# UMEssen/Body-and-Organ-Analysis

Hardware: AMD Instinct MI355X
Metric: CT volumes/sec (512^3 @1.5 mm, total+bca) on MI355X (higher is better)
Workload: dtype f16

## Files before the change

body-and-organ-analysis_amd/csrc/api.hip:

```cpp
#include <stdarg.h>
#include <stdlib.h>
#include <algorithm>
#include <iterator>
#include <string.h>

#include "common.h"

static thread_local char g_err[1024] = "";

void boa_set_error(const char* fmt, ...) {
    va_list ap;
    va_start(ap, fmt);
    vsnprintf(g_err, sizeof(g_err), fmt, ap);
    va_end(ap);
}

extern "C" const char* boa_last_error(void) { return g_err; }
extern "C" int boa_version(void) { return 100; }

extern "C" int boa_init(int device, void* stream, boa_ctx** out) {
    BOA_REQUIRE(out != nullptr, "boa_init: out is NULL");
    int n = 0;
    BOA_HIP_TRY(hipGetDeviceCount(&n));
    BOA_REQUIRE(device >= 0 && device < n, "boa_init: device %d not available (%d visible)", device, n);
// ... 12 lines not shown
    for (int i = 0; i < 8; ++i) {
        BOA_HIP_TRY(hipEventCreate(&c->t0[i]));
        BOA_HIP_TRY(hipEventCreate(&c->t1[i]));
    }
    *out = c;
    return BOA_OK;
}

extern "C" void boa_destroy(boa_ctx* c) {
    if (!c) return;
    hipSetDevice(c->device);
    hipStreamSynchronize(c->stream);
    for (int i = 0; i < 8; ++i) {
        hipEventDestroy(c->t0[i]);
        hipEventDestroy(c->t1[i]);
    }
    for (auto& r : c->prof_pending) hipEventDestroy(r.ev);
    for (auto e : c->ev_pool) hipEventDestroy(e);
    for (auto& r : c->ws_runs) hipFree(r.second);
    for (auto& b : c->pool_free) hipFree(b.second);
    for (auto& b : c->pool_live) hipFree(b.first);
    if (c->stash) hipFree(c->stash);
    if (c->act_arena) hipFree(c->act_arena);
    if (c->own_stream) hipStreamDestroy(c->stream);
    delete c;
}

extern "C" int boa_device_info(boa_ctx* c, char* name, int name_len, int* cu_count, size_t* total_mem,
                               size_t* free_mem) {
    BOA_REQUIRE(c, "ctx is NULL");
    hipDeviceProp_t p;
    BOA_HIP_TRY(hipGetDeviceProperties(&p, c->device));
    if (name && name_len > 0) {
        snprintf(name, name_len, "%s (%s)", p.name, p.gcnArchName);
    }
    if (cu_count) *cu_count = p.multiProcessorCount;
    size_t f = 0, t = 0;
    BOA_HIP_TRY(hipMemGetInfo(&f, &t));
    if (total_mem) *total_mem = t;
    if (free_mem) *free_mem = f;
    return BOA_OK;
}

int boa_malloc_raw(boa_ctx* c, size_t bytes, void** dev_out) {
    BOA_REQUIRE(c && dev_out, "boa_malloc: NULL argument");
    BOA_HIP_TRY(hipSetDevice(c->device));
// ... 65 lines not shown
            BOA_HIP_TRY(hipFree(last->second));
            c->pool_bytes -= last->first;
            c->pool_free.erase(last);
        }
    }
    return BOA_OK;
}

static int trim_locked(boa_ctx* c);
extern "C" int boa_trim(boa_ctx* c) {
    BOA_REQUIRE(c, "ctx is NULL");
    std::lock_guard<std::recursive_mutex> lock(c->pool_mu);
    return trim_locked(c);
}

extern "C" int boa_bind_thread(boa_ctx* c) {
    BOA_REQUIRE(c, "ctx is NULL");
    BOA_HIP_TRY(hipSetDevice(c->device));
    return BOA_OK;
}

static int trim_locked(boa_ctx* c) {
    const bool drop_stash = c->stash && !c->stash_busy;
    if (c->pool_free.empty() && !drop_stash && c->ws_desc_bytes == 0) return BOA_OK;
    BOA_HIP_TRY(hipStreamSynchronize(c->stream));
    for (size_t i = c->ws_runs.size(); i-- > 0;)
        if (!c->ws_runs[i].first.empty() && c->ws_runs[i].first[0] == -1) {
            hipFree(c->ws_runs[i].second);
            c->ws_runs.erase(c->ws_runs.begin() + i);
            c->ws_runs_host.erase(c->ws_runs_host.begin() + i);
        }
    c->ws_desc_bytes = 0;
    for (auto& b : c->pool_free) hipFree(b.second);
    c->pool_free.clear();
    c->pool_bytes = 0;
    if (drop_stash) {
        hipFree(c->stash);
        c->stash = nullptr;
        c->stash_bytes = 0;
    }
    return BOA_OK;
}

extern "C" int boa_memset(boa_ctx* c, void* dev, int value, size_t bytes) {
    BOA_REQUIRE(c && dev, "boa_memset: NULL argument");
    KernelTimer t(c, BOA_K_OTHER, 0, (double)bytes);
    BOA_HIP_TRY(hipMemsetAsync(dev, value, bytes, c->stream));
    t.stop();
// ... 71 lines not shown

KernelTimer::KernelTimer(boa_ctx* c, int kclass, double flops, double bytes) : ctx(c), k(kclass) {
    if (!c->prof) return;
    if (c->prof_pending.size() >= 32768) boa_prof_flush(c);
    on = true;
    c->prof_flops[k] += flops;
    c->prof_bytes[k] += bytes;
    c->prof_launches[k] += 1;
    if (c->prof_break || c->prof_pending.empty()) {
        hipEvent_t e = take_event(c);
        hipEventRecord(e, c->stream);
        c->prof_pending.push_back({-1, e});
        c->prof_break = false;
    }
}

void KernelTimer::stop() {
    if (!on) return;
    hipEvent_t e = take_event(ctx);
    hipEventRecord(e, ctx->stream);
    ctx->prof_pending.push_back({k, e});
}

int boa_prof_flush(boa_ctx* c) {
    if (!c->prof_pending.empty()) hipEventSynchronize(c->prof_pending.back().ev);
    for (size_t i = 0; i < c->prof_pending.size(); ++i) {
        const ProfRec& r = c->prof_pending[i];
        float ms = 0.f;
        if (r.kclass >= 0 && i > 0 && hipEventElapsedTime(&ms, c->prof_pending[i - 1].ev, r.ev) == hipSuccess)
            c->prof_ms[r.kclass] += ms;
        c->ev_pool.push_back(r.ev);
    }
    c->prof_pending.clear();
    c->prof_break = true;
    return BOA_OK;
}

extern "C" long long boa_debug_counter(boa_ctx* c, int which, int reset) {
    if (!c || which < 0 || which >= BOA_CNT_COUNT) return -1;
    const long long v = c->counters[which];
    if (reset) c->counters[which] = 0;
    return v;
}

extern "C" int boa_prof_enable(boa_ctx* c, int on) {
    BOA_REQUIRE(c, "ctx is NULL");
    if (!on) boa_prof_flush(c);
    c->prof = on != 0;
    return BOA_OK;
}

extern "C" int boa_prof_reset(boa_ctx* c) {
    BOA_REQUIRE(c, "ctx is NULL");
    boa_prof_flush(c);
    for (int i = 0; i < BOA_K_COUNT; ++i) {
        c->prof_ms[i] = 0;
        c->prof_launches[i] = 0;
// ... 17 lines not shown
```

body-and-organ-analysis_amd/csrc/comm.hip:

```cpp
#include <dlfcn.h>
#include <stdlib.h>
#include <string.h>
#include <rccl/rccl.h>

#include <algorithm>
#include <string>

#include "common.h"

namespace {

struct Rccl {
    void* h = nullptr;
    ncclResult_t (*GetUniqueId)(ncclUniqueId*) = nullptr;
    ncclResult_t (*CommInitRank)(ncclComm_t*, int, ncclUniqueId, int) = nullptr;
    ncclResult_t (*CommDestroy)(ncclComm_t) = nullptr;
    ncclResult_t (*Send)(const void*, size_t, ncclDataType_t, int, ncclComm_t, hipStream_t) = nullptr;
    ncclResult_t (*Recv)(void*, size_t, ncclDataType_t, int, ncclComm_t, hipStream_t) = nullptr;
    ncclResult_t (*AllReduce)(const void*, void*, size_t, ncclDataType_t, ncclRedOp_t, ncclComm_t, hipStream_t) = nullptr;
    ncclResult_t (*GroupStart)() = nullptr;
    ncclResult_t (*GroupEnd)() = nullptr;
    const char* (*GetErrorString)(ncclResult_t) = nullptr;
    std::string path;
};
// ... 91 lines not shown
    BOA_REQUIRE(ctx && id_in && out && world >= 1 && rank >= 0 && rank < world, "boa_comm_create: bad argument (world %d, rank %d)", world, rank);
    Rccl* R = rccl();
    BOA_REQUIRE(R, "boa_comm: librccl.so not found (set BOA_RCCL_LIB)");
    BOA_HIP_TRY(hipSetDevice(ctx->device));
    boa_comm* c = new boa_comm;
    c->ctx = ctx;
    c->world = world;
    c->rank = rank;
    ncclUniqueId id;
    memcpy(&id, id_in, 128);
    ncclResult_t r = R->CommInitRank(&c->comm, world, id, rank);
    if (r != ncclSuccess) {
        boa_set_error("ncclCommInitRank(world %d, rank %d) failed: %s", world, rank, R->GetErrorString ? R->GetErrorString(r) : "?");
        delete c;
        return BOA_EHIP;
    }
    if (hipStreamCreateWithFlags(&c->stream, hipStreamNonBlocking) != hipSuccess || hipEventCreateWithFlags(&c->ev_in, hipEventDisableTiming) != hipSuccess ||
        hipEventCreateWithFlags(&c->ev_out, hipEventDisableTiming) != hipSuccess) {
        boa_set_error("boa_comm_create: stream / event creation failed");
        R->CommDestroy(c->comm);
        delete c;
        return BOA_EHIP;
    }
    *out = c;
    return BOA_OK;
}

extern "C" void boa_comm_destroy(boa_comm* c) {
    if (!c) return;
    Rccl* R = rccl();
    if (c->stream) hipStreamSynchronize(c->stream);
    if (R && c->comm) R->CommDestroy(c->comm);
    if (c->ev_in) hipEventDestroy(c->ev_in);
    if (c->ev_out) hipEventDestroy(c->ev_out);
    if (c->stream) hipStreamDestroy(c->stream);
    delete c;
}

static int fence_in(boa_comm* c) {
    BOA_HIP_TRY(hipEventRecord(c->ev_in, c->ctx->stream));
    BOA_HIP_TRY(hipStreamWaitEvent(c->stream, c->ev_in, 0));
    return BOA_OK;
}

static int fence_out(boa_comm* c) {
    BOA_HIP_TRY(hipEventRecord(c->ev_out, c->stream));
// ... 150 lines not shown
```

body-and-organ-analysis_amd/csrc/common.h:

```cpp
#pragma once
#include <hip/hip_runtime.h>
#include <hip/hip_fp16.h>
#include <stdint.h>
#include <stdio.h>
#include <map>
#include <unordered_map>
#include <mutex>
#include <vector>

#include "boa_hip.h"

void boa_set_error(const char* fmt, ...);

#define BOA_HIP_TRY(expr)                                                                       \
    do {                                                                                        \
        hipError_t _e = (expr);                                                                 \
        if (_e != hipSuccess) {                                                                 \
            boa_set_error("%s failed: %s (%s:%d)", #expr, hipGetErrorString(_e), __FILE__, __LINE__); \
            return (_e == hipErrorOutOfMemory) ? BOA_ENOMEM : BOA_EHIP;                         \
        }                                                                                       \
    } while (0)

#define BOA_REQUIRE(cond, ...)                \
    do {                                      \
        if (!(cond)) {                        \
            boa_set_error(__VA_ARGS__);       \
            return BOA_EINVAL;                \
        }                                     \
    } while (0)
// ... 18 lines not shown
    bool prof = false;
    bool prof_break = true;
    std::vector<ProfRec> prof_pending;
    std::vector<hipEvent_t> ev_pool;
    double prof_ms[BOA_K_COUNT] = {};
    long long prof_launches[BOA_K_COUNT] = {};
    double prof_flops[BOA_K_COUNT] = {};
    double prof_bytes[BOA_K_COUNT] = {};
    long long counters[BOA_CNT_COUNT] = {};
    std::vector<std::pair<std::vector<int>, void*>> ws_runs;
    std::vector<std::vector<int>> ws_runs_host;
    size_t ws_desc_bytes = 0;
    std::recursive_mutex pool_mu;
    std::multimap<size_t, void*> pool_free;
    std::unordered_map<void*, size_t> pool_live;
    size_t pool_bytes = 0;
    size_t pool_cap = 0;
    void* stash = nullptr;
    size_t stash_bytes = 0;
    bool stash_busy = false;
    void* act_arena = nullptr;
    size_t act_bytes = 0;
    unsigned long long act_gen = 0;
};
int boa_malloc_raw(boa_ctx* c, size_t bytes, void** dev_out);

struct KernelTimer {
    boa_ctx* ctx;
    int k;
    bool on = false;
    KernelTimer(boa_ctx* c, int kclass, double flops, double bytes);
    void stop();
};
int boa_prof_flush(boa_ctx* ctx);

static inline int ceil_div(int a, int b) { return (a + b - 1) / b; }

__device__ __forceinline__ void idx3(size_t i, int d1, int d2, int& o0, int& o1, int& o2) {
    if (i <= 0xffffffffull) {
        const unsigned u = (unsigned)i, r = u / (unsigned)d2;
        o2 = (int)(u - r * (unsigned)d2);
        o0 = (int)(r / (unsigned)d1);
        o1 = (int)(r - (unsigned)o0 * (unsigned)d1);
    } else {
        const size_t r = i / (size_t)d2;
        o2 = (int)(i - r * (size_t)d2);
        o0 = (int)(r / (size_t)d1);
// ... 9 lines not shown
```

body-and-organ-analysis_amd/csrc/conv_ws.hip:

```cpp
#include <stdlib.h>

#include "conv.h"
#include "conv_ws_dev.h"

__global__ __launch_bounds__(64) void k_ws_build_desc(ConvArgs p, int grid, int row, int* __restrict__ out) {
    const int b = (int)blockIdx.x * 64 + (int)threadIdx.x;
    if (b >= grid) return;
    int* r = out + (size_t)b * row * 8;
    int my = 0;
    for (int v = b; v < p.N * p.vw; v += grid) my += p.runs[(v % p.vw) * 8];
    if (my > row - 1) my = row - 1;
    r[0] = my;
    for (int i = 1; i < 8; ++i) r[i] = 0;
    TileSeq s;
    s.n = s.left = s.j = 0;
    for (int k = 0; k < my; ++k) {
        bool new_run = true;
        if (k == 0)
            seq_first_of(p, s, b);
        else
            new_run = seq_next(p, s);
        const TileDesc d = make_desc(p, s, new_run);
        int* e = r + (size_t)(k + 1) * 8;
        e[0] = d.tc.n; e[1] = d.tc.cy; e[2] = d.tc.ox0; e[3] = d.tc.oy0; e[4] = d.tc.oz0; e[5] = d.flags; e[6] = d.vo; e[7] = d.ibase;
// ... 758 lines not shown
    const int vper = (a.N * a.vw + grid - 1) / grid;
    const int row = vper * (tiles_per_sample / a.vw + 2) + 1;
    *row_out = row;
    for (auto& e : ctx->ws_runs)
        if (e.first == key) return (const int*)e.second;
    {
        const std::vector<int>* runs_host = nullptr;
        for (size_t i = 0; i < ctx->ws_runs.size(); ++i)
            if (ctx->ws_runs[i].second == (const void*)a.runs) runs_host = &ctx->ws_runs_host[i];
        if (!runs_host || runs_host->size() < (size_t)a.vw * 8) return nullptr;
        for (int b = 0; b < grid; ++b) {
            long long my = 0;
            for (long long v = b; v < (long long)a.N * a.vw; v += grid) my += (*runs_host)[(size_t)(v % a.vw) * 8];
            if (my > row - 1) {
                boa_set_error("conv_ws: workgroup %d walks %lld tiles, descriptor rows hold %d", b, my, row - 1);
                return nullptr;
            }
        }
    }
    void* dev = nullptr;
    const size_t bytes = (size_t)grid * row * 8 * sizeof(int);
    if (hipMalloc(&dev, bytes) != hipSuccess) return nullptr;
    hipLaunchKernelGGL(k_ws_build_desc, dim3((grid + 63) / 64), dim3(64), 0, ctx->stream, a, grid, row, (int*)dev);
    ctx->ws_runs.emplace_back(std::move(key), dev);
    ctx->ws_runs_host.emplace_back();
    ctx->ws_desc_bytes += bytes;
    return (const int*)dev;
}

int launch_conv_ws(boa_ctx* ctx, const ConvArgs& a_in, const ConvTile& t, double flops, double bytes, bool x3) {
    const ConvArgs& a0 = a_in;
    const int total = t.tiles[0] * t.tiles[1] * t.tiles[2] * (a0.Cout / 32);
    const int vw = conv_ws_vw(total, ctx->cu_count);
    const int grid = (int)std::min<long long>((long long)vw * a0.N, ctx->cu_count);
    const int taps = a0.k0 * a0.k1 * a0.k2;
    const int HV = t.h[0] * (t.xs > 0 ? t.xs : t.h[1] * t.h[2]);
    const int resident = conv_ws_resident(HV, taps, (a0.C0 + a0.C1) / 16, a0.Cout) ? 1 : 0;
    BOA_REQUIRE(!x3 || a0.Cout * 4 <= 2048, "conv_ws (split precision): Cout %d exceeds the 512-entry bias table kept in LDS behind the halo buffers", a0.Cout);
    BOA_REQUIRE((double)a0.Di * a0.Hi * a0.Wi <= 16777216.0 && std::max(a0.C0, a0.C1) * 2 < 16777216,
                "conv_ws: more than 2^24 input voxels per sample (24-bit offset multiply)");
    BOA_REQUIRE((double)a0.Di * a0.Hi * a0.Wi * std::max(a0.C0, a0.C1) * 2.0 < 4294967296.0,
                "conv_ws: one sample of the input exceeds 4 GiB (32-bit voxel offsets)");
#ifdef WS_WITH_TRACE
    static const bool want_trace = getenv("BOA_WS_TRACE") != nullptr;
#else
    static const bool want_trace = false;
// ... 62 lines not shown
```

body-and-organ-analysis_amd/csrc/net.h:

```cpp
#pragma once
#include <vector>

#include "conv.h"
#include "tile_grid.h"

enum class NetMode : int { F16 = 0, F32Ref = 1, Split = 2 };

struct ActLayout {
    int C;
    int esz;
    bool planar;
    size_t rec() const { return planar ? 32 : (size_t)C * esz; }
    size_t bytes(size_t vox) const { return vox * C * esz; }
    size_t tile(size_t i, size_t vox) const { return i * bytes(vox); }
    size_t skip(int n, size_t plane) const { return (size_t)n * plane * rec(); }
    size_t plane_stride(size_t vox) const { return planar ? vox : 0; }
    hipError_t copy_head(unsigned char* dst, const void* tile, int dp, size_t plane, size_t vox, hipStream_t s) const {
        const size_t n = (size_t)dp * plane * rec();
        const int planes = planar ? C * esz / 32 : 1;
        hipError_t e = hipSuccess;
        for (int k = 0; k < planes && e == hipSuccess; ++k)
            e = hipMemcpyAsync(dst + k * n, (const unsigned char*)tile + k * vox * rec(), n, hipMemcpyDeviceToDevice, s);
        return e;
    }
    int to_nchw(boa_ctx* c, const void* tile, const float* ss, float slope, size_t vox, float* out) const {
// ... 1 lines not shown
        if (esz == 4) return launch_octet_to_nchw_f32(c, (const float*)tile, ss, slope, C, vox, out);
        return launch_ndhwc_to_nchw_f32(c, (const __half*)tile, ss, slope, 1, C, vox, out);
    }
};

inline ActLayout act_layout(NetMode m, int C) { return {C, m == NetMode::F16 ? 2 : 4, m != NetMode::F32Ref}; }

struct ConvLayer {
    ConvGeom g{};
    ConvTile t{};
    int Cin0 = 0, Cin1 = 0;
    bool first = false;
    __half* wpk = nullptr;
    float* wfirst = nullptr;
    float* w32 = nullptr;
    float wscale = 1.f;
    float *bias = nullptr, *gamma = nullptr, *beta = nullptr;
    void* act = nullptr;
    float* partials = nullptr;
    float* ss = nullptr;
    unsigned* ss16 = nullptr;
    int nblk = 0;
    size_t w_elems = 0;
};

struct UpLayer {
    int Cin = 0, Cout = 0;
    int s[3] = {1, 1, 1};
    int din[3] = {0, 0, 0};
    __half* wpk = nullptr;
    float* w32 = nullptr;
    float* bias = nullptr;
    void* act = nullptr;
    float wscale = 1.f;
    float fold = 1.f;
};

constexpr int TILE_REF_BATCH = 16;

struct boa_net {
    boa_ctx* ctx = nullptr;
    boa_net_desc d{};
    int maxN = 1;
    NetMode mode = NetMode::F16;
    int mirror_mask = 0;
    float* mirror_tmp = nullptr;
    float* mirror_sum = nullptr;
    float* tiles32 = nullptr;
    std::vector<std::vector<ConvLayer>> enc;
    std::vector<UpLayer> up;
    std::vector<std::vector<ConvLayer>> dec;
    float *head_w = nullptr, *head_b = nullptr;
    int* dev_origins = nullptr;
    float* first_padded = nullptr;
    std::vector<void*> allocs;
    struct ActSlot {
        void** where;
        size_t offset;
    };
    std::vector<ActSlot> act_slots;
    size_t act_need = 0;
    unsigned long long act_gen_seen = 0;
    int dims[BOA_MAX_STAGES][3];
    struct WeightSet {
        const float* key;
        size_t n;
        unsigned long long sample_hash;
        unsigned char* arena;
        std::vector<float> scales;
    };
    std::vector<WeightSet> wsets;
};

int net_bind_arena(boa_net* net);
int net_forward_stack(boa_net* net, const float* volume, const int V[3], const int vol_off[3], const int* host_origins, int N, int flip_mask = 0);
int head_kernel(const boa_net* net);
int scatter_head(const boa_net* net, const void* act, const float* ss, const int P[3], size_t plane_stride, const float* w, const float* b,
                 float* logits_out, const uint16_t* gauss, uint16_t* acc, uint16_t* nacc, const int PV[3], const int start[3]);
int net_head(boa_net* net, int i, const int P[3], int plane_skip, float* logits_out, const uint16_t* gauss, uint16_t* acc, uint16_t* nacc,
             const int PV[3], const int start[3]);
int check_padded(const boa_net* net, const int V[3], const int PV[3], const int off[3], const char* who);
void conv_kernel_info(const boa_net* net, const ConvLayer& L, int info[3]);
void convt_kernel_info(const boa_net* net, const UpLayer& U, int info[3]);
```

body-and-organ-analysis_amd/csrc/net.hip:

```cpp
#include <math.h>
#include <stdlib.h>
#include <string.h>

#include <vector>

#include "net.h"

namespace {

int in_granule(NetMode m) { return m == NetMode::F16 ? 16 : m == NetMode::Split ? 8 : 0; }

enum class Piece {
    FirstW,
    ConvW16,
    ConvWX3,
    ConvW32,
    Bias, Gamma, Beta,
    UpW16,
    UpWX3,
    UpW32,
    UpBias,
    HeadW, HeadB,
};

Piece conv_weight_piece(NetMode m, bool first) {
    if (m == NetMode::F32Ref) return Piece::ConvW32;
    if (first) return Piece::FirstW;
    return m == NetMode::Split ? Piece::ConvWX3 : Piece::ConvW16;
}

Piece convt_weight_piece(NetMode m) { return m == NetMode::F32Ref ? Piece::UpW32 : m == NetMode::Split ? Piece::UpWX3 : Piece::UpW16; }

}

static int net_alloc(boa_net* net, size_t bytes, void** out) {
    BOA_TRY(boa_malloc_raw(net->ctx, bytes, out));
    net->allocs.push_back(*out);
    return BOA_OK;
}

static int net_alloc_act(boa_net* net, size_t bytes, void** out) {
    *out = nullptr;
    net->act_slots.push_back({out, net->act_need});
    net->act_need += (bytes + 255) & ~(size_t)255;
    return BOA_OK;
}

int net_bind_arena(boa_net* net) {
    boa_ctx* c = net->ctx;
    if (net->act_slots.empty()) return BOA_OK;
    if (c->act_bytes < net->act_need) {
        BOA_HIP_TRY(hipStreamSynchronize(c->stream));
        if (c->act_arena) hipFree(c->act_arena);
        c->act_arena = nullptr;
        c->act_bytes = 0;
        BOA_TRY(boa_malloc_raw(c, net->act_need, &c->act_arena));
        c->act_bytes = net->act_need;
        c->act_gen++;
    }
    if (net->act_gen_seen != c->act_gen) {
        for (auto& sl : net->act_slots) *sl.where = (unsigned char*)c->act_arena + sl.offset;
        net->act_gen_seen = c->act_gen;
    }
    return BOA_OK;
}

static bool desc_ok(const boa_net_desc* d) {
    if (!d || d->n_stages < 2 || d->n_stages > BOA_MAX_STAGES || d->in_channels < 1 || d->num_classes < 1) return false;
    for (int s = 0; s < d->n_stages; ++s) {
        if (d->features[s] <= 0 || d->n_conv_enc[s] < 1) return false;
        for (int a = 0; a < 3; ++a)
            if ((d->kernel[s][a] != 1 && d->kernel[s][a] != 3) || d->stride[s][a] < 1 || d->stride[s][a] > 2) return false;
    }
    for (int s = 0; s < d->n_stages - 1; ++s)
        if (d->n_conv_dec[s] < 1) return false;
    return true;
}

extern "C" size_t boa_net_weight_count(const boa_net_desc* d) {
    if (!desc_ok(d)) return 0;
    size_t n = 0;
    int cin = d->in_channels;
    for (int s = 0; s < d->n_stages; ++s) {
        int taps = d->kernel[s][0] * d->kernel[s][1] * d->kernel[s][2];
        for (int i = 0; i < d->n_conv_enc[s]; ++i) {
            n += (size_t)d->features[s] * cin * taps + 3 * (size_t)d->features[s];
            cin = d->features[s];
// ... 31 lines not shown
        int p = (k[a] - 1) / 2;
        dout[a] = (din[a] + 2 * p - k[a]) / s[a] + 1;
    }
    L.g.Do = dout[0]; L.g.Ho = dout[1]; L.g.Wo = dout[2];
    const int taps = k[0] * k[1] * k[2];
    L.w_elems = (size_t)cout * (cin0 + cin1) * taps;
    const int gran = in_granule(net->mode);
    if (gran == 0) {
        BOA_REQUIRE(cout % 32 == 0, "conv %d+%d -> %d: Cout must be a multiple of 32", cin0, cin1, cout);
    } else if (first) {
        BOA_REQUIRE(s[0] == 1 && s[1] == 1 && s[2] == 1, "first conv must have stride 1");
        BOA_REQUIRE(cout % 32 == 0 && cin0 >= 1 && cin0 <= 4, "first conv %d -> %d unsupported", cin0, cout);
        L.nblk = conv_first_nblk(dout, net->ctx->cu_count);
    } else {
        BOA_REQUIRE((cin0 % gran) == 0 && (cin1 % gran) == 0 && (cout % 32) == 0,
                    "conv %d+%d -> %d: channel counts must be multiples of %d (in) / 32 (out)", cin0, cin1, cout, gran);
        ConvGeom gref = L.g;
        gref.N = TILE_REF_BATCH;
        BOA_REQUIRE(choose_conv_tile(gref, net->ctx->cu_count, &L.t, gran == 8), "no tile configuration fits conv %dx%dx%d k=%dx%dx%d",
                    din[0], din[1], din[2], k[0], k[1], k[2]);
        L.nblk = conv_nblk(L.t, net->ctx->cu_count, cout);
    }
    const ActLayout lay = act_layout(net->mode, cout);
    BOA_TRY(net_alloc_act(net, N * lay.bytes((size_t)dout[0] * dout[1] * dout[2]), &L.act));
    if (gran) {
        BOA_TRY(net_alloc(net, (size_t)N * cout * 2 * L.nblk * sizeof(float), (void**)&L.partials));
        BOA_HIP_TRY(hipMemsetAsync(L.partials, 0, (size_t)N * cout * 2 * L.nblk * sizeof(float), net->ctx->stream));
    }
    BOA_TRY(net_alloc(net, (size_t)N * cout * 2 * sizeof(float), (void**)&L.ss));
    if (lay.esz == 2)
        BOA_TRY(net_alloc(net, (size_t)N * cout * sizeof(unsigned), (void**)&L.ss16));
    return BOA_OK;
}

template <typename F>
static void for_each_weight_piece(boa_net* net, F&& f) {
    auto conv = [&](ConvLayer& L) {
        const int cin = L.Cin0 + L.Cin1, cout = L.g.Cout;
        const Piece w = conv_weight_piece(net->mode, L.first);
        f(w, &L, nullptr, w == Piece::ConvWX3   ? conv_wpk_halves_x3(cin, cout, L.g.k) * sizeof(__half)
                          : w == Piece::ConvW16 ? conv_wpk_halves(cin, cout, L.g.k) * sizeof(__half)
                                                : L.w_elems * sizeof(float));
        f(Piece::Bias, &L, nullptr, cout * sizeof(float));
        f(Piece::Gamma, &L, nullptr, cout * sizeof(float));
        f(Piece::Beta, &L, nullptr, cout * sizeof(float));
    };
    for (auto& st : net->enc)
// ... 211 lines not shown
    net->up.resize(d.n_stages - 1);
    net->dec.resize(d.n_stages - 1);
    for (int k = 0; k < d.n_stages - 1; ++k) {
        int sb = d.n_stages - 1 - k;
        UpLayer& U = net->up[k];
        U.Cin = d.features[sb];
        U.Cout = d.features[sb - 1];
        for (int a = 0; a < 3; ++a) {
            U.s[a] = d.stride[sb][a];
            U.din[a] = net->dims[sb][a];
        }
        int dup[3] = {U.din[0] * U.s[0], U.din[1] * U.s[1], U.din[2] * U.s[2]};
        for (int a = 0; a < 3; ++a)
            if (dup[a] != net->dims[sb - 1][a]) {
                boa_set_error("decoder %d: upsampled dim %d (%d) != skip dim (%d); patch not divisible by strides", k, a,
                              dup[a], net->dims[sb - 1][a]);
                return fail(BOA_EINVAL);
            }
        const int gran = in_granule(net->mode);
        if ((gran && U.Cin % gran) || U.Cout % 32) {
            boa_set_error("transposed conv %d -> %d: unsupported channel counts", U.Cin, U.Cout);
            return fail(BOA_EINVAL);
        }
        if ((rc = net_alloc_act(net, max_batch * act_layout(net->mode, U.Cout).bytes((size_t)dup[0] * dup[1] * dup[2]), &U.act)))
            return fail(rc);
        net->dec[k].resize(d.n_conv_dec[k]);
        int one[3] = {1, 1, 1};
        for (int i = 0; i < d.n_conv_dec[k]; ++i) {
            int c0 = U.Cout, c1 = (i == 0) ? U.Cout : 0;
            rc = setup_conv(net, net->dec[k][i], max_batch, dup, c0, c1, U.Cout, d.kernel[sb - 1], one, false);
            if (rc) return fail(rc);
        }
    }
    if ((rc = net_alloc(net, (size_t)max_batch * 3 * sizeof(int), (void**)&net->dev_origins))) return fail(rc);
    if (net->mode == NetMode::F32Ref) {
        if ((rc = net_alloc_act(net, (size_t)max_batch * d.in_channels * d.patch[0] * d.patch[1] * d.patch[2] * sizeof(float),
                                (void**)&net->tiles32)))
            return fail(rc);
    } else {
        int PD[3];
        conv_first_padded_dims(d.patch, d.kernel[0], PD);
        if ((rc = net_alloc_act(net, (size_t)max_batch * d.in_channels * PD[0] * PD[1] * PD[2] * sizeof(float),
                                (void**)&net->first_padded)))
            return fail(rc);
    }
    if ((rc = net_bind_arena(net))) return fail(rc);
    if (host_weights) {
        rc = boa_net_load_weights(net, host_weights, n_floats);
        if (rc) return fail(rc);
    }
    *out = net;
    return BOA_OK;
}


struct Fwd {
    const float* volume;
    const int* V;
    const int* vol_off;
    int N, flip_mask;
};

struct LayerProf {
    boa_ctx* c;
    int N;
    const char* tag;
// ... 228 lines not shown
        const bool last = k + 1 == combos.size();
        for (int i = 0; i < nb; ++i) {
            BOA_TRY(net_head(net, i, d.patch, 0, net->mirror_tmp + (size_t)i * per, nullptr, nullptr, nullptr, nullptr, nullptr));
            BOA_TRY(launch_flip_accumulate(net->ctx, net->mirror_tmp + (size_t)i * per, net->mirror_sum + (size_t)i * per, d.num_classes,
                                           d.patch, flip, k > 0, last ? (float)combos.size() : 1.0f));
        }
    }
    return BOA_OK;
}

extern "C" int boa_net_set_mirroring(boa_net* net, int axes_mask) {
    BOA_REQUIRE(net && axes_mask >= 0 && axes_mask < 8, "boa_net_set_mirroring: axes mask %d", axes_mask);
    net->mirror_mask = axes_mask;
    return BOA_OK;
}

extern "C" int boa_net_forward(boa_net* net, const float* dev_volume, const int V[3], const int* host_origins,
                               int n_tiles, float* dev_logits_out) {
    BOA_REQUIRE(net && dev_volume && V && host_origins && dev_logits_out, "boa_net_forward: NULL argument");
    BOA_TRY(net_bind_arena(net));
    const boa_net_desc& d = net->d;
    const size_t pv = (size_t)d.patch[0] * d.patch[1] * d.patch[2];
    const int zero[3] = {0, 0, 0};
    for (int t0 = 0; t0 < n_tiles; t0 += net->maxN) {
        int nb = std::min(net->maxN, n_tiles - t0);
        if (net->mirror_mask) {
            BOA_TRY(net_mirrored_logits(net, dev_volume, V, zero, host_origins + (size_t)t0 * 3, nb));
            BOA_HIP_TRY(hipMemcpyAsync(dev_logits_out + (size_t)t0 * d.num_classes * pv, net->mirror_sum,
                                       (size_t)nb * d.num_classes * pv * sizeof(float), hipMemcpyDeviceToDevice, net->ctx->stream));
            net->ctx->prof_break = true;
            continue;
        }
        BOA_TRY(net_forward_stack(net, dev_volume, V, zero, host_origins + (size_t)t0 * 3, nb));
        for (int i = 0; i < nb; ++i)
            BOA_TRY(net_head(net, i, d.patch, 0, dev_logits_out + (size_t)(t0 + i) * d.num_classes * pv, nullptr, nullptr, nullptr,
                             nullptr, nullptr));
    }
    return BOA_OK;
}

int check_padded(const boa_net* net, const int V[3], const int PV[3], const int off[3], const char* who) {
    for (int a = 0; a < 3; ++a)
        BOA_REQUIRE(PV[a] >= net->d.patch[a] && off[a] >= 0 && off[a] + V[a] <= PV[a],
                    "%s: padded dim %d (%d) must cover patch (%d) and volume (%d at %d)", who, a, PV[a], net->d.patch[a], V[a], off[a]);
    return BOA_OK;
}

extern "C" int boa_net_predict_sliding_window(boa_net* net, const float* dev_volume, const int V[3], const int PV[3],
                                              const int* vol_off, const int* host_origins, int n_tiles,
                                              const uint16_t* dev_gauss, uint16_t* dev_acc, uint16_t* dev_n) {
    BOA_REQUIRE(net && dev_volume && V && PV && host_origins && dev_acc && dev_n,
                "boa_net_predict_sliding_window: NULL argument");
    BOA_TRY(net_bind_arena(net));
    const boa_net_desc& d = net->d;
    const int zero[3] = {0, 0, 0};
    const int* off = vol_off ? vol_off : zero;
    BOA_TRY(check_padded(net, V, PV, off, "sliding window"));
    const size_t pv = (size_t)d.patch[0] * d.patch[1] * d.patch[2];
    for (int t0 = 0; t0 < n_tiles; t0 += net->maxN) {
        int nb = std::min(net->maxN, n_tiles - t0);
        if (net->mirror_mask) {
            BOA_TRY(net_mirrored_logits(net, dev_volume, V, off, host_origins + (size_t)t0 * 3, nb));
            for (int i = 0; i < nb; ++i)
                BOA_TRY(boa_accumulate_tile(net->ctx, net->mirror_sum + (size_t)i * d.num_classes * pv, dev_gauss, dev_acc, dev_n,
                                            d.num_classes, d.patch, PV, host_origins + (size_t)(t0 + i) * 3));
            continue;
        }
        BOA_TRY(net_forward_stack(net, dev_volume, V, off, host_origins + (size_t)t0 * 3, nb));
        for (int i = 0; i < nb; ++i) {
            const int* st = host_origins + (size_t)(t0 + i) * 3;
            BOA_TRY(net_head(net, i, d.patch, 0, nullptr, dev_gauss, dev_acc, dev_n, PV, st));
        }
    }
    return BOA_OK;
}
```

body-and-organ-analysis_amd/csrc/net_stash.hip:

```cpp
#include <stdlib.h>

#include <memory>

#include "net.h"

struct StashView {
    unsigned char* base = nullptr;
    StashOffsets o{};
    int ntile[3] = {0, 0, 0};
    bool x3 = false;
    float* ss() const { return (float*)(base + o.ss); }
    unsigned* ss16() const { return (unsigned*)(base + o.ss16); }
    unsigned* ssp() const { return (unsigned*)(base + o.ssp); }
    int* tab() const { return (int*)(base + o.tab); }
    int tiles() const { return ntile[0] * ntile[1] * ntile[2]; }
    size_t tab_ints(const int PV[3]) const { return walk_table_ints(ntile[0], ntile[1], ntile[2], PV); }
};

static GatherHead gather_head_on(const boa_net* net, const StashView& v, const int P[3], const int PV[3], const float* w, const float* b,
                                 const uint16_t* gauss) {
    GatherHead g;
    g.act = (const __half*)v.base; g.ssp = v.x3 ? (const unsigned*)v.ss() : v.ssp(); g.dev_tab = v.tab();
    g.tiles_total = v.tiles(); g.x3 = v.x3;
    g.w = w; g.bias = b; g.gauss = gauss; g.C = net->d.num_classes; g.slope = net->d.lrelu_slope;
// ... 32 lines not shown
        c->stash = nullptr;
        boa_set_error("fused sliding window: %zu bytes of stash do not fit", need);
        return BOA_ENOMEM;
    }
    c->stash_bytes = need;
    return BOA_OK;
}

static int net_forward_into_stash(boa_net* net, const float* dev_volume, const int V[3], const int PV[3], const int* off, const int* host_origins,
                                  int n_tiles, TileStash& ts) {
    boa_ctx* c = net->ctx;
    const boa_net_desc& d = net->d;
    grid_origins(host_origins, n_tiles, ts.steps);
    StashView& v = ts.v;
    for (int a = 0; a < 3; ++a) v.ntile[a] = (int)ts.steps[a].size();
    const int F0 = d.features[0];
    const size_t pv = (size_t)d.patch[0] * d.patch[1] * d.patch[2];
    const ActLayout lay = act_layout(net->mode, F0);
    v.o = stash_offsets(lay.tile(n_tiles, pv), n_tiles, F0, true, v.tab_ints(PV));
    BOA_TRY(reserve_ctx_stash(c, v.o.bytes));
    v.base = (unsigned char*)c->stash;
    v.x3 = lay.esz == 4;
    ConvLayer& last = net->dec.back().back();
    void* keep_act = last.act;
    float* keep_ss = last.ss;
    unsigned* keep_ss16 = last.ss16;
    int rc = BOA_OK;
    for (int t0 = 0; t0 < n_tiles && rc == BOA_OK; t0 += net->maxN) {
        const int nb = std::min(net->maxN, n_tiles - t0);
        last.act = v.base + lay.tile(t0, pv);
        last.ss = v.ss() + (size_t)t0 * F0 * 2;
        last.ss16 = keep_ss16 ? v.ss16() + (size_t)t0 * F0 : nullptr;
        rc = net_forward_stack(net, dev_volume, V, off, host_origins + (size_t)t0 * 3, nb);
    }
    last.act = keep_act;
    last.ss = keep_ss;
    last.ss16 = keep_ss16;
    if (rc) return rc;
    if (!v.x3) BOA_TRY(launch_pack_head_ss(c, v.ss(), v.ssp(), n_tiles));
    const std::vector<int> tab = walk_table(ts.steps[0], ts.steps[1], ts.steps[2], d.patch, PV);
    BOA_REQUIRE(tab.size() == v.tab_ints(PV), "walk table: %zu ints, %zu reserved", tab.size(), v.tab_ints(PV));
    BOA_HIP_TRY(hipMemcpyAsync(v.tab(), tab.data(), tab.size() * sizeof(int), hipMemcpyHostToDevice, c->stream));
    BOA_HIP_TRY(hipStreamSynchronize(c->stream));
    c->prof_break = true;
    return BOA_OK;
}

extern "C" int boa_net_labels_supported(boa_net* net, const int* host_origins, int n_tiles) {
    if (!net || !host_origins) return 0;
    if (!act_layout(net->mode, net->d.features[0]).planar || net->mirror_mask != 0 || net->d.features[0] != 32 || net->d.num_classes > 31 || net->d.patch[2] % 32 != 0) return 0;
    std::vector<int> steps[3];
    return grid_origins(host_origins, n_tiles, steps) ? 1 : 0;
}

extern "C" int boa_net_predict_labels_fold(boa_net* net, const float* dev_volume, const int V[3], const int PV[3], const int* vol_off,
                                           const int* host_origins, int n_tiles, const uint16_t* dev_gauss, uint16_t* dev_fold,
                                           int fold_index, int n_folds, const uint8_t* host_lut, int merge, uint8_t* dev_labels_out,
                                           const int* crop_off, const int* crop_dims, int* dev_inf_flag) {
    BOA_REQUIRE(net && dev_volume && V && PV && host_origins && dev_inf_flag, "boa_net_predict_labels_fold: NULL argument");
    BOA_REQUIRE(boa_net_labels_supported(net, host_origins, n_tiles), "boa_net_predict_labels_fold: unsupported network / tile layout");
    BOA_TRY(net_bind_arena(net));
// ... 207 lines not shown
```

include/boa_hip.h:

```cpp
#ifndef BOA_HIP_H
#define BOA_HIP_H

#include <stddef.h>
#include <stdint.h>

#ifdef __cplusplus
extern "C" {
#endif

#define BOA_OK 0
#define BOA_EINVAL (-1)
#define BOA_EHIP (-2)
#define BOA_ENOMEM (-3)
#define BOA_EINF (-4)

typedef struct boa_ctx boa_ctx;
typedef struct boa_net boa_net;

const char* boa_last_error(void);
int boa_version(void);
int boa_init(int device, void* stream, boa_ctx** out);
void boa_destroy(boa_ctx* ctx);
int boa_device_info(boa_ctx* ctx, char* name, int name_len, int* cu_count, size_t* total_mem, size_t* free_mem);
int boa_malloc(boa_ctx* ctx, size_t bytes, void** dev_out);
// ... 16 lines not shown
#define BOA_K_HEAD_ACCUM 4
#define BOA_K_ARGMAX 5
#define BOA_K_OTHER 6
#define BOA_K_AGG 7
#define BOA_K_MORPH 8
#define BOA_K_RESAMPLE 9
#define BOA_K_COPY 10
#define BOA_K_COUNT 11
int boa_prof_enable(boa_ctx* ctx, int on);
int boa_prof_reset(boa_ctx* ctx);
int boa_prof_get(boa_ctx* ctx, int kclass, double* total_ms, long long* launches, double* flops, double* bytes);
#define BOA_CNT_HEAD_MFMA 0
#define BOA_CNT_HEAD_VALU 1
#define BOA_CNT_CONV_WS 2
#define BOA_CNT_CONV_SIMPLE 3
#define BOA_CNT_FIRST_MFMA 4
#define BOA_CNT_FIRST_VALU 5
#define BOA_CNT_F32 6
#define BOA_CNT_CONV_X3 7
#define BOA_CNT_X3 8
#define BOA_CNT_HEAD_GATHER 9
#define BOA_CNT_COPY_T 10
#define BOA_CNT_BBOX_VEC 11
#define BOA_CNT_COUNT 12
long long boa_debug_counter(boa_ctx* ctx, int which, int reset);

int boa_ct_normalize(boa_ctx* ctx, const void* dev_in, int in_dtype, float* dev_out, size_t n,
                     float mean, float std, float lo, float hi);

int boa_accumulate_tile(boa_ctx* ctx, const float* dev_pred, const uint16_t* dev_gauss, uint16_t* dev_acc,
                        uint16_t* dev_n, int C, const int P[3], const int V[3], const int start[3]);

int boa_finalize_labels(boa_ctx* ctx, uint16_t* dev_acc, const uint16_t* dev_n, int C, const int V[3],
                        uint16_t* dev_fold_sum, int fold_mode, int n_folds_final, int write_logits,
                        const uint8_t* host_lut, int merge, uint8_t* dev_labels_out,
                        const int* crop_off, const int* crop_dims, int* dev_inf_flag);
int boa_finalize_labels_planes(boa_ctx* ctx, uint16_t* dev_acc, const uint16_t* dev_n, int C, const int V[3],
                               uint16_t* dev_fold_sum, int fold_mode, int n_folds_final, int write_logits,
                               const uint8_t* host_lut, int merge, uint8_t* dev_labels_out, const int* crop_off,
                               const int* crop_dims, int* dev_inf_flag, int plane_lo, int plane_hi);

#define BOA_MAX_STAGES 8
typedef struct {
    int n_stages;
    int in_channels;
    int num_classes;
    int features[BOA_MAX_STAGES];
// ... 319 lines not shown
```

Baseline: 0.5956.

## Run alternating tile batches on two streams with duplicated activation arenas

Adds a second HIP stream and a second activation arena, plus per-lane partials and stats buffers. Successive tile batches of the sliding-window forward alternate between the two lanes so that consecutive batches can overlap on the GPU. Ordered sections, the head accumulation into shared buffers, are serialized with events. The cost is double activation memory and added event synchronization. Two lanes are disabled under sharding, mirroring, F32 reference mode or low free memory.

New measurement: 0.6009, median of 6. Within noise of the previous version (+0.9%).

```diff
diff --git a/body-and-organ-analysis_amd/csrc/api.hip b/body-and-organ-analysis_amd/csrc/api.hip
--- a/body-and-organ-analysis_amd/csrc/api.hip
+++ b/body-and-organ-analysis_amd/csrc/api.hip
@@ -58,6 +58,14 @@
     for (auto& b : c->pool_live) hipFree(b.first);
     if (c->stash) hipFree(c->stash);
     if (c->act_arena) hipFree(c->act_arena);
+    if (c->lane_stream) {
+        hipStreamSynchronize(c->lane_stream);
+        hipStreamDestroy(c->lane_stream);
+    }
+    for (auto& r : c->lane_prof_pending) hipEventDestroy(r.ev);
+    for (hipEvent_t e : c->lane_ev)
+        if (e) hipEventDestroy(e);
+    if (c->act_arena1) hipFree(c->act_arena1);
     if (c->own_stream) hipStreamDestroy(c->stream);
     delete c;
 }
@@ -169,8 +177,16 @@
 
 static int trim_locked(boa_ctx* c) {
     const bool drop_stash = c->stash && !c->stash_busy;
-    if (c->pool_free.empty() && !drop_stash && c->ws_desc_bytes == 0) return BOA_OK;
+    const bool drop_arena1 = c->act_arena1 && !c->lanes_live;
+    if (c->pool_free.empty() && !drop_stash && !drop_arena1 && c->ws_desc_bytes == 0) return BOA_OK;
     BOA_HIP_TRY(hipStreamSynchronize(c->stream));
+    if (c->lane_stream) BOA_HIP_TRY(hipStreamSynchronize(c->lane_stream));
+    if (drop_arena1) {
+        hipFree(c->act_arena1);
+        c->act_arena1 = nullptr;
+        c->act_bytes1 = 0;
+        c->act_gen1++;
+    }
     for (size_t i = c->ws_runs.size(); i-- > 0;)
         if (!c->ws_runs[i].first.empty() && c->ws_runs[i].first[0] == -1) {
             hipFree(c->ws_runs[i].second);
@@ -288,17 +304,23 @@
     ctx->prof_pending.push_back({k, e});
 }
 
-int boa_prof_flush(boa_ctx* c) {
-    if (!c->prof_pending.empty()) hipEventSynchronize(c->prof_pending.back().ev);
-    for (size_t i = 0; i < c->prof_pending.size(); ++i) {
-        const ProfRec& r = c->prof_pending[i];
+static void prof_flush_chain(boa_ctx* c, std::vector<ProfRec>& pending) {
+    if (!pending.empty()) hipEventSynchronize(pending.back().ev);
+    for (size_t i = 0; i < pending.size(); ++i) {
+        const ProfRec& r = pending[i];
         float ms = 0.f;
-        if (r.kclass >= 0 && i > 0 && hipEventElapsedTime(&ms, c->prof_pending[i - 1].ev, r.ev) == hipSuccess)
+        if (r.kclass >= 0 && i > 0 && hipEventElapsedTime(&ms, pending[i - 1].ev, r.ev) == hipSuccess)
             c->prof_ms[r.kclass] += ms;
         c->ev_pool.push_back(r.ev);
     }
-    c->prof_pending.clear();
+    pending.clear();
+}
+
+int boa_prof_flush(boa_ctx* c) {
+    prof_flush_chain(c, c->prof_pending);
+    prof_flush_chain(c, c->lane_prof_pending);
     c->prof_break = true;
+    c->lane_prof_break = true;
     return BOA_OK;
 }
 
diff --git a/body-and-organ-analysis_amd/csrc/batch_lanes.h b/body-and-organ-analysis_amd/csrc/batch_lanes.h
--- /dev/null
+++ b/body-and-organ-analysis_amd/csrc/batch_lanes.h
@@ -0,0 +1,13 @@
+#pragma once
+#include <vector>
+
+inline int lane_count(int n_batches, bool two_lanes_allowed) { return two_lanes_allowed && n_batches >= 2 ? 2 : 1; }
+
+inline std::vector<int> lane_schedule(int n_batches, bool two_lanes_allowed) {
+    std::vector<int> out;
+    if (n_batches <= 0) return out;
+    const bool two = lane_count(n_batches, two_lanes_allowed) == 2;
+    out.reserve((size_t)n_batches);
+    for (int i = 0; i < n_batches; ++i) out.push_back(two ? (i & 1) : 0);
+    return out;
+}
diff --git a/body-and-organ-analysis_amd/csrc/comm.hip b/body-and-organ-analysis_amd/csrc/comm.hip
--- a/body-and-organ-analysis_amd/csrc/comm.hip
+++ b/body-and-organ-analysis_amd/csrc/comm.hip
@@ -137,6 +137,7 @@
         delete c;
         return BOA_EHIP;
     }
+    if (world > 1) ctx->sharded = true;
     *out = c;
     return BOA_OK;
 }
diff --git a/body-and-organ-analysis_amd/csrc/common.h b/body-and-organ-analysis_amd/csrc/common.h
--- a/body-and-organ-analysis_amd/csrc/common.h
+++ b/body-and-organ-analysis_amd/csrc/common.h
@@ -5,6 +5,7 @@
 #include <stdio.h>
 #include <map>
 #include <unordered_map>
+#include <utility>
 #include <mutex>
 #include <vector>
 
@@ -69,7 +70,24 @@
     void* act_arena = nullptr;
     size_t act_bytes = 0;
     unsigned long long act_gen = 0;
+    hipStream_t lane_stream = nullptr;
+    std::vector<ProfRec> lane_prof_pending;
+    bool lane_prof_break = true;
+    bool on_lane1 = false;
+    bool lanes_live = false;
+    bool sharded = false;
+    hipEvent_t lane_ev[4] = {};
+    void* act_arena1 = nullptr;
+    size_t act_bytes1 = 0;
+    unsigned long long act_gen1 = 0;
 };
+
+static inline void lane_swap(boa_ctx* c) {
+    std::swap(c->stream, c->lane_stream);
+    c->prof_pending.swap(c->lane_prof_pending);
+    std::swap(c->prof_break, c->lane_prof_break);
+    c->on_lane1 = !c->on_lane1;
+}
 int boa_malloc_raw(boa_ctx* c, size_t bytes, void** dev_out);
 
 struct KernelTimer {
diff --git a/body-and-organ-analysis_amd/csrc/conv_ws.hip b/body-and-organ-analysis_amd/csrc/conv_ws.hip
--- a/body-and-organ-analysis_amd/csrc/conv_ws.hip
+++ b/body-and-organ-analysis_amd/csrc/conv_ws.hip
@@ -804,6 +804,10 @@
     const size_t bytes = (size_t)grid * row * 8 * sizeof(int);
     if (hipMalloc(&dev, bytes) != hipSuccess) return nullptr;
     hipLaunchKernelGGL(k_ws_build_desc, dim3((grid + 63) / 64), dim3(64), 0, ctx->stream, a, grid, row, (int*)dev);
+    if (ctx->lanes_live && hipStreamSynchronize(ctx->stream) != hipSuccess) {
+        hipFree(dev);
+        return nullptr;
+    }
     ctx->ws_runs.emplace_back(std::move(key), dev);
     ctx->ws_runs_host.emplace_back();
     ctx->ws_desc_bytes += bytes;
diff --git a/body-and-organ-analysis_amd/csrc/net.h b/body-and-organ-analysis_amd/csrc/net.h
--- a/body-and-organ-analysis_amd/csrc/net.h
+++ b/body-and-organ-analysis_amd/csrc/net.h
@@ -1,6 +1,7 @@
 #pragma once
 #include <vector>
 
+#include "batch_lanes.h"
 #include "conv.h"
 #include "tile_grid.h"
 
@@ -48,6 +49,10 @@
     unsigned* ss16 = nullptr;
     int nblk = 0;
     size_t w_elems = 0;
+    void* act1 = nullptr;
+    float* partials1 = nullptr;
+    float* ss1 = nullptr;
+    unsigned* ss16_1 = nullptr;
 };
 
 struct UpLayer {
@@ -60,6 +65,7 @@
     void* act = nullptr;
     float wscale = 1.f;
     float fold = 1.f;
+    void* act1 = nullptr;
 };
 
 constexpr int TILE_REF_BATCH = 16;
@@ -87,6 +93,12 @@
     std::vector<ActSlot> act_slots;
     size_t act_need = 0;
     unsigned long long act_gen_seen = 0;
+    std::vector<ActSlot> act_slots1;
+    unsigned long long act_gen1_seen = 0;
+    bool lane1_ready = false;
+    bool on_lane1 = false;
+    int* dev_origins1 = nullptr;
+    float* first_padded1 = nullptr;
     int dims[BOA_MAX_STAGES][3];
     struct WeightSet {
         const float* key;
@@ -96,6 +108,21 @@
         std::vector<float> scales;
     };
     std::vector<WeightSet> wsets;
+};
+
+struct BatchLanes {
+    boa_net* net;
+    bool two = false, ordered = false;
+    std::vector<int> plan;
+    explicit BatchLanes(boa_net* n) : net(n) {}
+    ~BatchLanes();
+    BatchLanes(const BatchLanes&) = delete;
+    BatchLanes& operator=(const BatchLanes&) = delete;
+    int begin(int n_batches);
+    int select(int batch);
+    int end();
+    int ordered_begin();
+    int ordered_end();
 };
 
 int net_bind_arena(boa_net* net);
diff --git a/body-and-organ-analysis_amd/csrc/net.hip b/body-and-organ-analysis_amd/csrc/net.hip
--- a/body-and-organ-analysis_amd/csrc/net.hip
+++ b/body-and-organ-analysis_amd/csrc/net.hip
@@ -39,9 +39,13 @@
     return BOA_OK;
 }
 
-static int net_alloc_act(boa_net* net, size_t bytes, void** out) {
+static int net_alloc_act(boa_net* net, size_t bytes, void** out, void** out1) {
     *out = nullptr;
     net->act_slots.push_back({out, net->act_need});
+    if (out1) {
+        *out1 = nullptr;
+        net->act_slots1.push_back({out1, net->act_need});
+    }
     net->act_need += (bytes + 255) & ~(size_t)255;
     return BOA_OK;
 }
@@ -63,6 +67,152 @@
         net->act_gen_seen = c->act_gen;
     }
     return BOA_OK;
+}
+
+
+static int net_bind_lane1(boa_net* net) {
+    boa_ctx* c = net->ctx;
+    if (c->act_bytes1 < net->act_need) {
+        BOA_HIP_TRY(hipStreamSynchronize(c->stream));
+        if (c->lane_stream) BOA_HIP_TRY(hipStreamSynchronize(c->lane_stream));
+        if (c->act_arena1) hipFree(c->act_arena1);
+        c->act_arena1 = nullptr;
+        c->act_bytes1 = 0;
+        c->act_gen1++;
+        size_t fr = 0, tot = 0;
+        if (hipMemGetInfo(&fr, &tot) != hipSuccess || net->act_need > fr / 2) return BOA_ENOMEM;
+        if (hipMalloc(&c->act_arena1, net->act_need) != hipSuccess) {
+            (void)hipGetLastError();
+            c->act_arena1 = nullptr;
+            return BOA_ENOMEM;
+        }
+        c->act_bytes1 = net->act_need;
+        c->act_gen1++;
+    }
+    if (net->act_gen1_seen != c->act_gen1) {
+        for (auto& sl : net->act_slots1) *sl.where = (unsigned char*)c->act_arena1 + sl.offset;
+        net->act_gen1_seen = c->act_gen1;
+    }
+    if (net->lane1_ready) return BOA_OK;
+    auto conv = [&](ConvLayer& L) -> int {
+        const size_t N = (size_t)net->maxN, cout = (size_t)L.g.Cout;
+        if (L.partials && !L.partials1) {
+            BOA_TRY(net_alloc(net, N * cout * 2 * L.nblk * sizeof(float), (void**)&L.partials1));
+            BOA_HIP_TRY(hipMemsetAsync(L.partials1, 0, N * cout * 2 * L.nblk * sizeof(float), c->stream));
+        }
+        if (!L.ss1) BOA_TRY(net_alloc(net, N * cout * 2 * sizeof(float), (void**)&L.ss1));
+        if (L.ss16 && !L.ss16_1) BOA_TRY(net_alloc(net, N * cout * sizeof(unsigned), (void**)&L.ss16_1));
+        return BOA_OK;
+    };
+    for (auto& st : net->enc)
+        for (auto& L : st) BOA_TRY(conv(L));
+    for (auto& st : net->dec)
+        for (auto& L : st) BOA_TRY(conv(L));
+    if (!net->dev_origins1) BOA_TRY(net_alloc(net, (size_t)net->maxN * 3 * sizeof(int), (void**)&net->dev_origins1));
+    c->prof_break = true;
+    net->lane1_ready = true;
+    return BOA_OK;
+}
+
+static void net_swap_lane(boa_net* net) {
+    auto conv = [](ConvLayer& L) {
+        std::swap(L.act, L.act1);
+        std::swap(L.partials, L.partials1);
+        std::swap(L.ss, L.ss1);
+        std::swap(L.ss16, L.ss16_1);
+    };
+    for (auto& st : net->enc)
+        for (auto& L : st) conv(L);
+    for (auto& st : net->dec)
+        for (auto& L : st) conv(L);
+    for (auto& U : net->up) std::swap(U.act, U.act1);
+    std::swap(net->dev_origins, net->dev_origins1);
+    std::swap(net->first_padded, net->first_padded1);
+    net->on_lane1 = !net->on_lane1;
+}
+
+static bool layer_prof_on() {
+    static const bool v = getenv("BOA_LAYER_PROF") != nullptr;
+    return v;
+}
+
+int BatchLanes::begin(int n_batches) {
+    boa_ctx* c = net->ctx;
+    static const bool one_lane = getenv("BOA_BATCH_LANES") && atoi(getenv("BOA_BATCH_LANES")) == 1;
+    bool allowed = !one_lane && !c->sharded && !c->lanes_live && !c->on_lane1 && net->mirror_mask == 0 && net->mode != NetMode::F32Ref &&
+                   !layer_prof_on();
+    if (lane_count(n_batches, allowed) == 2) {
+        const int rc = net_bind_lane1(net);
+        if (rc == BOA_ENOMEM)
+            allowed = false;
+        else if (rc != BOA_OK)
+            return rc;
+    }
+    plan = lane_schedule(n_batches, allowed);
+    if (lane_count(n_batches, allowed) != 2) return BOA_OK;
+    if (!c->lane_stream) BOA_HIP_TRY(hipStreamCreateWithFlags(&c->lane_stream, hipStreamNonBlocking));
+    for (hipEvent_t& e : c->lane_ev)
+        if (!e) BOA_HIP_TRY(hipEventCreateWithFlags(&e, hipEventDisableTiming));
+    BOA_HIP_TRY(hipEventRecord(c->lane_ev[0], c->stream));
+    BOA_HIP_TRY(hipStreamWaitEvent(c->lane_stream, c->lane_ev[0], 0));
+    c->lane_prof_break = true;
+    c->lanes_live = true;
+    two = true;
+    return BOA_OK;
+}
+
+int BatchLanes::select(int batch) {
+    if (!two) return BOA_OK;
+    boa_ctx* c = net->ctx;
+    BOA_REQUIRE(batch >= 0 && batch < (int)plan.size(), "batch lanes: batch %d of %zu", batch, plan.size());
+    const bool lane1 = plan[batch] == 1;
+    if (lane1 != c->on_lane1) lane_swap(c);
+    if (lane1 != net->on_lane1) net_swap_lane(net);
+    if (lane1) c->counters[BOA_CNT_LANE1_BATCHES]++;
+    return BOA_OK;
+}
+
+int BatchLanes::end() {
+    if (!two) return BOA_OK;
+    boa_ctx* c = net->ctx;
+    if (c->on_lane1) lane_swap(c);
+    if (net->on_lane1) net_swap_lane(net);
+    two = false;
+    c->lanes_live = false;
+    BOA_HIP_TRY(hipEventRecord(c->lane_ev[1], c->lane_stream));
+    BOA_HIP_TRY(hipStreamWaitEvent(c->stream, c->lane_ev[1], 0));
+    c->prof_break = true;
+    return BOA_OK;
+}
+
+int BatchLanes::ordered_begin() {
+    boa_ctx* c = net->ctx;
+    if (!two || !c->on_lane1) return BOA_OK;
+    BOA_HIP_TRY(hipEventRecord(c->lane_ev[2], c->stream));
+    lane_swap(c);
+    BOA_HIP_TRY(hipStreamWaitEvent(c->stream, c->lane_ev[2], 0));
+    c->prof_break = true;
+    ordered = true;
+    return BOA_OK;
+}
+
+int BatchLanes::ordered_end() {
+    if (!ordered) return BOA_OK;
+    boa_ctx* c = net->ctx;
+    ordered = false;
+    BOA_HIP_TRY(hipEventRecord(c->lane_ev[3], c->stream));
+    BOA_HIP_TRY(hipStreamWaitEvent(c->lane_stream, c->lane_ev[3], 0));
+    c->lane_prof_break = true;
+    return BOA_OK;
+}
+
+BatchLanes::~BatchLanes() {
+    if (!two) return;
+    boa_ctx* c = net->ctx;
+    if (c->on_lane1) lane_swap(c);
+    if (net->on_lane1) net_swap_lane(net);
+    c->lanes_live = false;
+    hipStreamSynchronize(c->lane_stream);
 }
 
 static bool desc_ok(const boa_net_desc* d) {
@@ -140,7 +290,7 @@
         L.nblk = conv_nblk(L.t, net->ctx->cu_count, cout);
     }
     const ActLayout lay = act_layout(net->mode, cout);
-    BOA_TRY(net_alloc_act(net, N * lay.bytes((size_t)dout[0] * dout[1] * dout[2]), &L.act));
+    BOA_TRY(net_alloc_act(net, N * lay.bytes((size_t)dout[0] * dout[1] * dout[2]), &L.act, &L.act1));
     if (gran) {
         BOA_TRY(net_alloc(net, (size_t)N * cout * 2 * L.nblk * sizeof(float), (void**)&L.partials));
         BOA_HIP_TRY(hipMemsetAsync(L.partials, 0, (size_t)N * cout * 2 * L.nblk * sizeof(float), net->ctx->stream));
@@ -398,7 +548,7 @@
             boa_set_error("transposed conv %d -> %d: unsupported channel counts", U.Cin, U.Cout);
             return fail(BOA_EINVAL);
         }
-        if ((rc = net_alloc_act(net, max_batch * act_layout(net->mode, U.Cout).bytes((size_t)dup[0] * dup[1] * dup[2]), &U.act)))
+        if ((rc = net_alloc_act(net, max_batch * act_layout(net->mode, U.Cout).bytes((size_t)dup[0] * dup[1] * dup[2]), &U.act, &U.act1)))
             return fail(rc);
         net->dec[k].resize(d.n_conv_dec[k]);
         int one[3] = {1, 1, 1};
@@ -411,13 +561,13 @@
     if ((rc = net_alloc(net, (size_t)max_batch * 3 * sizeof(int), (void**)&net->dev_origins))) return fail(rc);
     if (net->mode == NetMode::F32Ref) {
         if ((rc = net_alloc_act(net, (size_t)max_batch * d.in_channels * d.patch[0] * d.patch[1] * d.patch[2] * sizeof(float),
-                                (void**)&net->tiles32)))
+                                (void**)&net->tiles32, nullptr)))
             return fail(rc);
     } else {
         int PD[3];
         conv_first_padded_dims(d.patch, d.kernel[0], PD);
         if ((rc = net_alloc_act(net, (size_t)max_batch * d.in_channels * PD[0] * PD[1] * PD[2] * sizeof(float),
-                                (void**)&net->first_padded)))
+                                (void**)&net->first_padded, (void**)&net->first_padded1)))
             return fail(rc);
     }
     if ((rc = net_bind_arena(net))) return fail(rc);
@@ -692,8 +842,11 @@
     const boa_net_desc& d = net->d;
     const size_t pv = (size_t)d.patch[0] * d.patch[1] * d.patch[2];
     const int zero[3] = {0, 0, 0};
+    BatchLanes lanes(net);
+    BOA_TRY(lanes.begin((n_tiles + net->maxN - 1) / net->maxN));
     for (int t0 = 0; t0 < n_tiles; t0 += net->maxN) {
         int nb = std::min(net->maxN, n_tiles - t0);
+        BOA_TRY(lanes.select(t0 / net->maxN));
         if (net->mirror_mask) {
             BOA_TRY(net_mirrored_logits(net, dev_volume, V, zero, host_origins + (size_t)t0 * 3, nb));
             BOA_HIP_TRY(hipMemcpyAsync(dev_logits_out + (size_t)t0 * d.num_classes * pv, net->mirror_sum,
@@ -706,7 +859,7 @@
             BOA_TRY(net_head(net, i, d.patch, 0, dev_logits_out + (size_t)(t0 + i) * d.num_classes * pv, nullptr, nullptr, nullptr,
                              nullptr, nullptr));
     }
-    return BOA_OK;
+    return lanes.end();
 }
 
 int check_padded(const boa_net* net, const int V[3], const int PV[3], const int off[3], const char* who) {
@@ -727,8 +880,11 @@
     const int* off = vol_off ? vol_off : zero;
     BOA_TRY(check_padded(net, V, PV, off, "sliding window"));
     const size_t pv = (size_t)d.patch[0] * d.patch[1] * d.patch[2];
+    BatchLanes lanes(net);
+    BOA_TRY(lanes.begin((n_tiles + net->maxN - 1) / net->maxN));
     for (int t0 = 0; t0 < n_tiles; t0 += net->maxN) {
         int nb = std::min(net->maxN, n_tiles - t0);
+        BOA_TRY(lanes.select(t0 / net->maxN));
         if (net->mirror_mask) {
             BOA_TRY(net_mirrored_logits(net, dev_volume, V, off, host_origins + (size_t)t0 * 3, nb));
             for (int i = 0; i < nb; ++i)
@@ -737,10 +893,12 @@
             continue;
         }
         BOA_TRY(net_forward_stack(net, dev_volume, V, off, host_origins + (size_t)t0 * 3, nb));
+        BOA_TRY(lanes.ordered_begin());
         for (int i = 0; i < nb; ++i) {
             const int* st = host_origins + (size_t)(t0 + i) * 3;
             BOA_TRY(net_head(net, i, d.patch, 0, nullptr, dev_gauss, dev_acc, dev_n, PV, st));
         }
-    }
-    return BOA_OK;
-}
+        BOA_TRY(lanes.ordered_end());
+    }
+    return lanes.end();
+}
diff --git a/body-and-organ-analysis_amd/csrc/net_stash.hip b/body-and-organ-analysis_amd/csrc/net_stash.hip
--- a/body-and-organ-analysis_amd/csrc/net_stash.hip
+++ b/body-and-organ-analysis_amd/csrc/net_stash.hip
@@ -78,21 +78,24 @@
     v.base = (unsigned char*)c->stash;
     v.x3 = lay.esz == 4;
     ConvLayer& last = net->dec.back().back();
-    void* keep_act = last.act;
-    float* keep_ss = last.ss;
-    unsigned* keep_ss16 = last.ss16;
-    int rc = BOA_OK;
-    for (int t0 = 0; t0 < n_tiles && rc == BOA_OK; t0 += net->maxN) {
+    BatchLanes lanes(net);
+    BOA_TRY(lanes.begin((n_tiles + net->maxN - 1) / net->maxN));
+    for (int t0 = 0; t0 < n_tiles; t0 += net->maxN) {
         const int nb = std::min(net->maxN, n_tiles - t0);
+        BOA_TRY(lanes.select(t0 / net->maxN));
+        void* keep_act = last.act;
+        float* keep_ss = last.ss;
+        unsigned* keep_ss16 = last.ss16;
         last.act = v.base + lay.tile(t0, pv);
         last.ss = v.ss() + (size_t)t0 * F0 * 2;
         last.ss16 = keep_ss16 ? v.ss16() + (size_t)t0 * F0 : nullptr;
-        rc = net_forward_stack(net, dev_volume, V, off, host_origins + (size_t)t0 * 3, nb);
-    }
-    last.act = keep_act;
-    last.ss = keep_ss;
-    last.ss16 = keep_ss16;
-    if (rc) return rc;
+        const int rc = net_forward_stack(net, dev_volume, V, off, host_origins + (size_t)t0 * 3, nb);
+        last.act = keep_act;
+        last.ss = keep_ss;
+        last.ss16 = keep_ss16;
+        if (rc) return rc;
+    }
+    BOA_TRY(lanes.end());
     if (!v.x3) BOA_TRY(launch_pack_head_ss(c, v.ss(), v.ssp(), n_tiles));
     const std::vector<int> tab = walk_table(ts.steps[0], ts.steps[1], ts.steps[2], d.patch, PV);
     BOA_REQUIRE(tab.size() == v.tab_ints(PV), "walk table: %zu ints, %zu reserved", tab.size(), v.tab_ints(PV));
diff --git a/include/boa_hip.h b/include/boa_hip.h
--- a/include/boa_hip.h
+++ b/include/boa_hip.h
@@ -62,7 +62,8 @@
 #define BOA_CNT_HEAD_GATHER 9
 #define BOA_CNT_COPY_T 10
 #define BOA_CNT_BBOX_VEC 11
-#define BOA_CNT_COUNT 12
+#define BOA_CNT_LANE1_BATCHES 12
+#define BOA_CNT_COUNT 13
 long long boa_debug_counter(boa_ctx* ctx, int which, int reset);
 
 int boa_ct_normalize(boa_ctx* ctx, const void* dev_in, int in_dtype, float* dev_out, size_t n,
```
